# MarvinLvn/CPC2

Measured on AMD Instinct MI355X. Metric: audio-seconds/sec CPC training (1.28 s @16 kHz, 128 neg), higher is better.
Workload: dtype f32

## Files before the change

### cpc2_amd/_lib.py

```python
import ctypes
import os
import time

import torch

_HERE = os.path.dirname(os.path.abspath(__file__))
LIB_PATH = os.environ.get("CPC2_HIP_LIB") or os.path.join(_HERE, "libcpc2_hip.so")

c_float_p = ctypes.c_void_p
c_ptr = ctypes.c_void_p
c_int = ctypes.c_int
c_long = ctypes.c_long
c_size_t = ctypes.c_size_t
c_float = ctypes.c_float

SIGNATURES = {
    "cpc_version": (c_int, []),
    "cpc_last_error": (ctypes.c_char_p, []),
    "cpc_async_error_check": (c_int, [c_ptr]),
    "cpc_prof_enable": (c_int, [c_int]),
    "cpc_gemm_set_mode": (c_int, [c_int]),
    "cpc_prof_read": (c_int, [ctypes.c_char_p, ctypes.POINTER(ctypes.c_double), ctypes.POINTER(c_long)]),
    "cpc_gemm_nt": (c_int, [c_ptr, c_long, c_ptr, c_long, c_ptr, c_long, c_ptr, c_int, c_int, c_int, c_ptr]),
    "cpc_gemm_tn_scratch_bytes": (c_size_t, [c_int, c_int, c_long]),
# ... 51 lines not shown
    "cpc_mt_draw_host": (c_int, [c_ptr, c_ptr, c_size_t]),
    "cpc_mt_draw_host_async": (c_int, [c_ptr, c_ptr, c_size_t]),
    "cpc_mt_draw_device_async": (c_int, [c_ptr, c_ptr, c_ptr, c_size_t, c_int, c_ptr]),
    "cpc_mt_draw_expand_device_async": (c_int, [c_ptr, c_ptr, c_ptr, c_ptr, c_int, c_int, c_int, c_int, c_int, c_ptr]),
    "cpc_mt_redraw_expand_device_async": (c_int, [c_ptr, c_ptr, c_int, c_int, c_size_t, c_ptr, c_ptr, c_ptr, c_int, c_int, c_int, c_int, c_int, c_ptr]),
    "cpc_negidx_wait_on": (c_int, [c_ptr, c_ptr]),
    "cpc_negidx_stream": (c_int, [c_ptr, c_ptr]),
    "cpc_stream_create_apart": (c_int, [c_ptr, c_int, c_ptr]),
    "cpc_streams_overlap": (c_int, [c_ptr, c_ptr]),
    "cpc_stream_apart_failures": (c_long, []),
    "cpc_stream_spin": (c_int, [c_ptr, c_long]),
    "cpc_side_stream": (c_int, [c_ptr, c_ptr]),
    "cpc_negidx_expand": (c_int, [c_ptr, c_ptr, c_int, c_int, c_int, c_int, c_ptr]),
    "cpc_infonce_saved_bytes": (c_size_t, [c_int] * 6),
    "cpc_infonce_scratch_bytes": (c_size_t, [c_int] * 6),
    "cpc_infonce_logits_offset": (c_size_t, [c_int] * 6),
    "cpc_infonce_perm_offset": (c_size_t, [c_int] * 6),
    "cpc_infonce_forward": (c_int, [c_ptr] * 9 + [c_int] * 6 + [c_ptr]),
    "cpc_infonce_backward": (c_int, [c_ptr] * 11 + [c_int] * 6 + [c_ptr]),
    "cpc_infonce_backward_deferred": (c_int, [c_ptr] * 11 + [c_int] * 6 + [c_ptr]),
    "cpc_infonce_join": (c_int, [c_ptr]),
    "cpc_infonce_forward_cw": (c_int, [c_ptr] * 9 + [c_int] * 6 + [c_ptr]),
    "cpc_infonce_backward_cw": (c_int, [c_ptr] * 11 + [c_int] * 7 + [c_ptr]),
    "cpc_infonce_forward_pred": (c_int, [c_ptr] * 8 + [c_int] * 5 + [c_ptr]),
    "cpc_infonce_backward_pred": (c_int, [c_ptr] * 9 + [c_int] * 5 + [c_ptr]),
    "cpc_flac_info": (c_int, [ctypes.c_char_p, ctypes.POINTER(c_int), ctypes.POINTER(c_int), ctypes.POINTER(c_int),
                              ctypes.POINTER(c_long)]),
    "cpc_flac_decode_f32": (c_int, [ctypes.c_char_p, c_ptr, c_long, ctypes.POINTER(c_int)]),
    "cpc_window_gather": (c_int, [c_ptr, c_long, c_ptr, c_ptr, c_int, c_int, c_ptr]),
    "cpc_adam_step": (c_int, [c_ptr, c_ptr, c_ptr, c_ptr, c_long, c_int, c_float, c_float, c_float, c_float, c_float, c_ptr]),
# ... 121 lines not shown
```

### cpc2_amd/criterion.py

```python
import ctypes
import os

import numpy as np
import torch
import torch.nn as nn

from . import _lib
from ._lib import check, f32c, grad_buffers, ptr, require_gpu, scratch, stream_ptr


def _sleep_until(event):
    import time
    while not event.query():
        time.sleep(0.0001)


class NegativeSampler:

    RING = int(os.environ.get("CPC_SAMPLER_RING", "4"))

    def __init__(self):
        self._lib = _lib.load()
        self._h = ctypes.c_void_p(self._lib.cpc_mt_create(5489))
        if not self._h:
# ... 443 lines not shown
    def forward(ctx, z, ext_idx, weights, n_neg, *preds):
        require_gpu(z, ext_idx, weights, *preds)
        lib = _lib.load()
        z = f32c(z)
        preds = tuple(f32c(p) for p in preds)
        b, t, dim_enc = z.shape
        k = len(preds)
        if any(p.shape != (b, t - k, dim_enc) for p in preds):
            raise ValueError(f"predictions must be [b, W, dim_enc] = {(b, t - k, dim_enc)}")
        if ext_idx.dtype != torch.int32 or ext_idx.numel() != b * n_neg * (t - k):
            raise ValueError("ext_idx must be int32 [b, W, n_neg]")
        if weights is not None and weights.numel() != b * (t - k):
            raise ValueError(f"weights must hold one value per (window, frame): {b * (t - k)}, got {weights.numel()}")
        w = f32c(weights) if weights is not None else None
        nsaved = lib.cpc_infonce_saved_bytes(b, t, k, dim_enc, dim_enc, n_neg)
        nscratch = lib.cpc_infonce_scratch_bytes(b, t, k, dim_enc, dim_enc, n_neg)
        if nsaved == 0:
            check(-1, "infonce shape query")
        losses = torch.empty(k, dtype=torch.float32, device=z.device)
        acc = torch.empty(k, dtype=torch.float32, device=z.device)
        saved = torch.empty(nsaved, dtype=torch.uint8, device=z.device)
        sc = scratch(nscratch, z.device)
        check(lib.cpc_infonce_forward_pred(_lib.ptr_array(preds), ptr(z), ptr(ext_idx), ptr(w), ptr(losses), ptr(acc),
                                           ptr(saved), ptr(sc), b, t, k, dim_enc, n_neg, stream_ptr(z.device)),
              "infonce_forward_pred")
        ctx.save_for_backward(z, ext_idx, w, saved, *preds)
        ctx.dims = (b, t, k, dim_enc, n_neg)
        ctx.mark_non_differentiable(acc)
        ctx.set_materialize_grads(False)
        return losses, acc

    @staticmethod
    def backward(ctx, dlosses, _dacc):
        lib = _lib.load()
        z, ext_idx, w, saved, *preds = ctx.saved_tensors
        b, t, k, dim_enc, n_neg = ctx.dims
        if dlosses is None:
            dlosses = torch.zeros(k, dtype=torch.float32, device=z.device)
        dlosses = f32c(dlosses)
        dz = torch.empty_like(z)
        dpreds = [torch.empty_like(p) for p in preds]
        sc = scratch(lib.cpc_infonce_scratch_bytes(b, t, k, dim_enc, dim_enc, n_neg), z.device)
        check(lib.cpc_infonce_backward_pred(_lib.ptr_array(preds), ptr(z), ptr(ext_idx), ptr(w), ptr(dlosses), ptr(saved),
                                            ptr(sc), _lib.ptr_array(dpreds), ptr(dz), b, t, k, dim_enc, n_neg,
                                            stream_ptr(z.device)), "infonce_backward_pred")
        return (dz, None, None, None) + tuple(dpreds)


class _LinearFn(torch.autograd.Function):

    @staticmethod
    def forward(ctx, x, weight):
        require_gpu(x, weight)
        lib = _lib.load()
        x2 = f32c(x).reshape(-1, x.shape[-1])
        w = f32c(weight.detach())
        m, kdim = x2.shape
# ... 184 lines not shown
    def _logits(self, cFeature, encodedData, extIdx, n_neg):
        lib = _lib.load()
        with torch.no_grad():
            windowSize = cFeature.size(1) - self.nPredicts
            preds = self._predictions(cFeature[:, :windowSize].contiguous())
            z = f32c(encodedData)
            b, t, dim_enc = z.shape
            k = self.nPredicts
            losses = torch.empty(k, dtype=torch.float32, device=z.device)
            acc = torch.empty(k, dtype=torch.float32, device=z.device)
            dim_ar = dim_enc if preds is not None else cFeature.size(2)
            nsaved = lib.cpc_infonce_saved_bytes(b, t, k, dim_ar, dim_enc, n_neg)
            if nsaved == 0:
                check(-1, "infonce shape query")
            saved = torch.empty(nsaved, dtype=torch.uint8, device=z.device)
            sc = scratch(lib.cpc_infonce_scratch_bytes(b, t, k, dim_ar, dim_enc, n_neg), z.device)
            if preds is None:
                c = f32c(cFeature)
                wpred = torch.stack([f32c(p.weight.detach()) for p in self.wPrediction.predictors], dim=0)
                check(lib.cpc_infonce_forward(ptr(c), ptr(z), ptr(wpred), ptr(extIdx), None, ptr(losses), ptr(acc), ptr(saved),
                                              ptr(sc), b, t, k, dim_ar, dim_enc, n_neg, stream_ptr(z.device)), "infonce_forward")
            else:
                preds = [f32c(p) for p in preds]
                check(lib.cpc_infonce_forward_pred(_lib.ptr_array(preds), ptr(z), ptr(extIdx), None, ptr(losses), ptr(acc),
                                                   ptr(saved), ptr(sc), b, t, k, dim_enc, n_neg, stream_ptr(z.device)),
                      "infonce_forward_pred")
            off = lib.cpc_infonce_logits_offset(b, t, k, dim_ar, dim_enc, n_neg)
            n = b * windowSize * k * (n_neg + 1)
            slot_order = saved[off:off + 4 * n].view(torch.float32).view(b, windowSize, k, n_neg + 1)
            poff = lib.cpc_infonce_perm_offset(b, t, k, dim_ar, dim_enc, n_neg)
            perm = saved[poff:poff + 2 * b * windowSize * n_neg].view(torch.int16).view(b, windowSize, 1, n_neg).long() & 0xFFFF
# ... 246 lines not shown
```

### cpc2_amd/csrc/infonce.hip

```cpp
#include "common.h"
#include <hip/hip_ext.h>
#include "coop.h"
#include "ldsdma.h"
#include "rowcfg.h"

#include <algorithm>
#include <atomic>
#include <cstdlib>
#include <map>
#include <mutex>

namespace cpc {

typedef float f32x4 __attribute__((ext_vector_type(4)));
typedef float f32x16 __attribute__((ext_vector_type(16)));

constexpr int NCE_ROWS = 16;
constexpr int NCE_POS = 16;

struct NceArgs {
    const float *Pk[16];
    float *dPk[16];
    long p_stride;
    int p_rows;
    int p_packed;
    const float *z;
    const int32_t *ext;
    const unsigned short *perm;
    const float *weights;
    float *logits;
    float *lse;
    float *lossp;
    float *hit;
    int b, T, W, K, Nneg;
    int lw;
    const float *dloss;
    float *vbuf;
    float *ds_buf;
    float inv_count;
};

__global__ __launch_bounds__(64) void nce_block_sort_kernel(const int32_t *ext, int32_t *sorted, unsigned short *perm, int Nneg,
                                                            int rows_per_block, int nblk, int nrows, int *err)
{
    const long base = (long)blockIdx.x * Nneg;
    const int lane = threadIdx.x;
    int pos = 0;
    bool bad = false;
    for (int blk = 0; blk < nblk; ++blk)
        for (int c = 0; c < Nneg; c += 64) {
            const int j = c + lane;
            int row = j < Nneg ? ext[base + j] : -1;
            if (j < Nneg && (unsigned)row >= (unsigned)nrows) { bad = true; row = 0; }
// ... 483 lines not shown
#pragma unroll
        for (int dt = 0; dt < DT32; ++dt) {
            f32x16 acc;
#pragma unroll
            for (int e = 0; e < 16; ++e) acc[e] = 0.f;
#pragma unroll
            for (int kp = 0; kp < NCE_ROWS / 2; ++kp) acc = __builtin_amdgcn_mfma_f32_32x32x2f32(av[kp], bvals[dt][kp], acc, 0, 0, 0);
#pragma unroll
            for (int e = 0; e < 16; ++e)
                if (voff[e] >= 0) vb[voff[e] + dt * 32] = acc[e];
        }
    }
}

constexpr int NCE_SROW = 68;
template <int H, int NKK> __global__ __launch_bounds__(H / 2) void infonce_bwd_fused_kernel(NceArgs a)
{
    constexpr int NW = H / 128;
    extern __shared__ __attribute__((aligned(16))) float smem[];
    float *dS = smem;
    int *rowidx = reinterpret_cast<int *>(dS + NCE_ROWS * a.lw);
    float *stage0 = reinterpret_cast<float *>(rowidx + a.lw);
    const int wave = threadIdx.x >> 6, lane = threadIdx.x & 63, r = lane & 15, q = lane >> 4;
    float *stage = stage0 + wave * 16 * NCE_SROW;

    const int bb = blockIdx.x / a.p_rows, t = blockIdx.x - bb * a.p_rows;
    if (t >= a.W) {
        for (int k = 0; k < a.K; ++k) {
            float *row = a.dPk[k] + ((long)bb * a.p_rows + t) * a.p_stride;
            for (int i = threadIdx.x; i < H / 4; i += 64 * NW) reinterpret_cast<float4 *>(row)[i] = make_float4(0.f, 0.f, 0.f, 0.f);
        }
// ... 40 lines not shown
    }
    __syncthreads();
#pragma unroll
    for (int kk = 0; kk < KW; ++kk) {
        const int k = wave + NW * kk, kc = min(k, a.K - 1);
#pragma unroll
        for (int i = 0; i < GI; ++i) {
            const int g = lane + 64 * i;
            const float e = expf(stage0[kc * lrow + gi[i]] - lsek[kk]);
            float v = g >= NCE_POS ? (g < ncand ? coef[kk] * e : 0.f) : (g == k ? coef[kk] * (e - 1.f) : 0.f);
            if (k >= a.K) v = 0.f;
            if (g < a.lw) dS[k * a.lw + g] = v;
        }
    }
    __syncthreads();

    const int d0 = 128 * wave;
    const long prow_off = ((long)bb * a.p_rows + t) * a.p_stride + d0;
    float pa[8][NKK];
#pragma unroll
    for (int kk = 0; kk < NKK; ++kk) {
        const int k = 4 * kk + q;
        const float *pk = a.Pk[min(k, a.K - 1)] + prow_off + r;
#pragma unroll
        for (int tile = 0; tile < 8; ++tile) {
            const float v = pk[16 * tile];
            pa[tile][kk] = k < a.K ? v : 0.f;
        }
    }
    float *vb = a.vbuf + (bt * (long)ncand + q) * H + d0 + 4 * r;
#define NCE_ROWS_GROUP(C0)                                                                                                     \
    {                                                                                                                          \
        const int c0_ = (C0);                                                                                                  \
        float bv[NKK];                                                                                                         \
        _Pragma("unroll") for (int kk = 0; kk < NKK; ++kk) bv[kk] = dS[(4 * kk + q) * a.lw + c0_ + r];                        \
        _Pragma("unroll") for (int half = 0; half < 2; ++half) {                                                               \
            f32x4 acc[4];                                                                                                      \
            _Pragma("unroll") for (int tl = 0; tl < 4; ++tl) acc[tl] = (f32x4){0.f, 0.f, 0.f, 0.f};                            \
            _Pragma("unroll") for (int kk = 0; kk < NKK; ++kk)                                                                 \
                _Pragma("unroll") for (int tl = 0; tl < 4; ++tl)                                                               \
                    acc[tl] = __builtin_amdgcn_mfma_f32_16x16x4f32(pa[4 * half + tl][kk], bv[kk], acc[tl], 0, 0, 0);           \
            _Pragma("unroll") for (int tl = 0; tl < 4; ++tl)                                                                   \
                *reinterpret_cast<f32x4 *>(stage + r * NCE_SROW + 16 * tl + 4 * q) = acc[tl];                                  \
            __builtin_amdgcn_fence(__ATOMIC_RELEASE, "wavefront");                                                             \
            __builtin_amdgcn_wave_barrier();                                                                                   \
// ... 29 lines not shown
        auto multiply = [&](int buf) {
#pragma unroll
            for (int u = 0; u < 4; ++u)
#pragma unroll
                for (int T4 = 0; T4 < 2; ++T4) {
                    dp[T4][0] = __builtin_amdgcn_mfma_f32_16x16x4f32(av[buf][u][T4].x, bv4[buf][u], dp[T4][0], 0, 0, 0);
                    dp[T4][1] = __builtin_amdgcn_mfma_f32_16x16x4f32(av[buf][u][T4].y, bv4[buf][u], dp[T4][1], 0, 0, 0);
                    dp[T4][2] = __builtin_amdgcn_mfma_f32_16x16x4f32(av[buf][u][T4].z, bv4[buf][u], dp[T4][2], 0, 0, 0);
                    dp[T4][3] = __builtin_amdgcn_mfma_f32_16x16x4f32(av[buf][u][T4].w, bv4[buf][u], dp[T4][3], 0, 0, 0);
                }
        };
        const int nb = npad / 16;
        request(0, 0);
        for (int ib = 0; ib < nb; ib += 2) {
            request(1, 4 * (ib + 1));
            NCE_ROWS_GROUP(16 * ib)
            multiply(0);
            if (ib + 2 < nb) request(0, 4 * (ib + 2));
            if (16 * (ib + 1) < ncand) NCE_ROWS_GROUP(16 * (ib + 1))
            multiply(1);
        }
        if (r < a.K) {
            float *dprow = a.dPk[r] + ((long)bb * a.p_rows + t) * a.p_stride + d0;
#pragma unroll
            for (int T4 = 0; T4 < 2; ++T4)
#pragma unroll
                for (int reg = 0; reg < 4; ++reg)
                    *reinterpret_cast<float4 *>(dprow + 64 * T4 + 16 * q + 4 * reg) =
                        make_float4(dp[T4][0][reg], dp[T4][1][reg], dp[T4][2][reg], dp[T4][3][reg]);
        }
    }
#undef NCE_ROWS_GROUP
}

// ... 101 lines not shown
    }
    for (; e > beg; --e) {
        const int o = entries[e - 1];
        add_row((long)(o / Nneg) * vrows + pos_rows + o % Nneg);
    }
    for (int k = 0; k < K; ++k) {
        const int t = tp - 1 - k;
        if (t >= 0 && t < W) add_row(((long)bb * W + t) * vrows + k);
    }
#pragma unroll
    for (int c = 0; c < PER; ++c)
        if (lane + 64 * c < C4) reinterpret_cast<float4 *>(dz)[(long)r * C4 + lane + 64 * c] = acc[c];
    }
}

__global__ void negidx_expand_kernel(const uint32_t *raw, int32_t *ext, int b, int T, int W, int Nneg)
{
    const long n = (long)b * Nneg * W;
    for (long o = (long)blockIdx.x * blockDim.x + threadIdx.x; o < n; o += (long)gridDim.x * blockDim.x) {
        const int nn = (int)(o % Nneg);
        const long bt = o / Nneg;
        const int t = (int)(bt % W), bb = (int)(bt / W);
        const long i = ((long)bb * Nneg + nn) * W + t;
        const uint32_t bi = raw[i] % (uint32_t)b;
        uint32_t seq = raw[n + i] % (uint32_t)(T - 1) + 1u + (uint32_t)t;
        if (seq >= (uint32_t)T) seq -= (uint32_t)T;
        ext[o] = (int32_t)(seq + bi * (uint32_t)T);
    }
}

struct NceLayout {
    int b, T, K, W, Har, Henc, Nneg, lw;
    int Pr;
    float *P, *logits, *lse;
    int32_t *ext_sorted;
    unsigned short *perm;
    int nblk, rows_per_block;
    size_t saved_bytes;
    float *lossp, *hit, *dP, *wt, *tn, *tn_late;
    float *vbuf;
    float *ds_buf;
    int *counts, *offsets, *entries;
    size_t tn_bytes, scratch_bytes;
    size_t lds_fwd, lds_bwd, lds_bwd_fused;
};

static bool nce_supported(int H) { return H == 32 || H == 64 || H == 128 || H == 256 || H == 512; }

static int nce_layout(NceLayout &l, int b, int T, int K, int Har, int Henc, int Nneg, void *saved, void *scratch)
{
    CPC_REQUIRE(nce_supported(Henc), "infonce: encoder dim %d not supported (32, 64, 128, 256, 512)", Henc);
    CPC_REQUIRE(b > 0 && K >= 1 && K <= 16 && T > K && Nneg >= 1 && Har >= 1,
                "infonce: bad shape b=%d T=%d K=%d (1..16) dim_ar=%d n_neg=%d", b, T, K, Har, Nneg);
    l.b = b; l.T = T; l.K = K; l.W = T - K; l.Har = Har; l.Henc = Henc; l.Nneg = Nneg; l.Pr = T;
    l.lw = (int)cdiv(NCE_POS + Nneg, 32) * 32 + 4;
    Carver sv(saved);
    l.P = sv.take<float>((size_t)b * T * K * Henc);
    l.logits = sv.take<float>((size_t)b * l.W * K * (Nneg + 1));
    l.lse = sv.take<float>((size_t)b * l.W * K);
    l.ext_sorted = sv.take<int32_t>((size_t)b * l.W * Nneg);
    l.perm = sv.take<unsigned short>((size_t)b * l.W * Nneg + 1024);
    const size_t zbytes = sizeof(float) * (size_t)b * T * Henc;
    l.nblk = (int)std::min<size_t>(16, std::max<size_t>(1, (zbytes + (1u << 21) - 1) >> 21));
    l.rows_per_block = (int)cdiv((long)b * T, l.nblk);
    l.saved_bytes = sv.used();
    Carver sc(scratch);
    l.lossp = sc.take<float>((size_t)b * l.W * K);
    l.hit = sc.take<float>((size_t)b * l.W * K);
    l.dP = sc.take<float>((size_t)b * T * K * Henc);
    l.wt = sc.take<float>((size_t)K * Henc * Har);
    l.tn_bytes = std::max(gemm_tn_scratch_bytes(K * Henc, Har, (long)b * T), gemm_nt_scratch_bytes((long)b * T, Har, K * Henc));
    l.tn = sc.take<float>(l.tn_bytes / sizeof(float));
    l.tn_late = sc.take<float>(l.tn_bytes / sizeof(float));
    l.counts = sc.take<int>((size_t)b * T);
    l.offsets = sc.take<int>((size_t)b * T + 1);
    l.entries = sc.take<int>((size_t)b * l.W * Nneg);
    l.vbuf = sc.take<float>((size_t)b * l.W * (NCE_POS + Nneg) * Henc);
    l.ds_buf = sc.take<float>((size_t)b * l.W * (NCE_ROWS + 1) * l.lw);
    l.scratch_bytes = sc.used();
    l.lds_fwd = align_up(sizeof(int) * (size_t)Nneg + sizeof(unsigned short) * (size_t)Nneg, 16);
    l.lds_bwd = sizeof(float) * (size_t)NCE_ROWS * l.lw + sizeof(int) * (size_t)l.lw;
    CPC_REQUIRE(l.lds_bwd <= 64 * 1024, "infonce: n_neg=%d needs %zu B of LDS (> 64 KiB)", Nneg, l.lds_bwd);
    l.lds_bwd_fused = l.lds_bwd + sizeof(float) * (size_t)(Henc / 128) * 16 * NCE_SROW;
    return CPC_OK;
}

template <typename Kern> static int allow_lds(Kern kern, size_t bytes)
{
    if (bytes > 64 * 1024)
        CPC_CHECK_HIP(hipFuncSetAttribute(reinterpret_cast<const void *>(kern), hipFuncAttributeMaxDynamicSharedMemorySize, (int)bytes));
    return CPC_OK;
}
// ... 87 lines not shown
    std::lock_guard<std::mutex> lk(mu);
    NceSide &sd = sides[dev];
    if (sd.stream == nullptr) {
        CPC_TRY(stream_create_apart(&caller, 1, &sd.stream));
        CPC_CHECK_HIP(hipEventCreateWithFlags(&sd.fork, hipEventDisableTiming));
        CPC_CHECK_HIP(hipEventCreateWithFlags(&sd.join, hipEventDisableTiming));
        CPC_CHECK_HIP(hipEventCreateWithFlags(&sd.mid, hipEventDisableTiming));
        CPC_CHECK_HIP(hipEventCreateWithFlags(&sd.late, hipEventDisableTiming));
        CPC_CHECK_HIP(hipEventCreateWithFlags(&sd.tail_fork, hipEventDisableTiming));
        CPC_CHECK_HIP(hipEventCreateWithFlags(&sd.tail, hipEventDisableTiming));
    }
    *out = &sd;
    return CPC_OK;
}

static int nce_launch_gather(const NceLayout &l, float *dz, bool fused, hipStream_t st)
{
    const int rows = l.b * l.T;
    const unsigned wgs = (unsigned)cdiv(rows, 4);
    NCE_DISPATCH(l.Henc, hipLaunchKernelGGL(infonce_dz_gather_kernel<HH>, dim3(wgs), dim3(256), 0, st, l.vbuf,
                                             l.offsets, l.entries, dz, l.b, l.T, l.W, l.K, l.Nneg, fused ? NCE_POS : l.K));
    CPC_CHECK_LAUNCH("infonce_dz_gather_kernel");
    return CPC_OK;
}

static int nce_launch_bwd(NceArgs &a, const NceLayout &l, float *dz, hipStream_t st, NceSide **late = nullptr)
{
    const long n = (long)l.b * l.W * l.Nneg;
    const int rows = l.b * l.T;
    a.vbuf = l.vbuf;
    a.ds_buf = l.ds_buf;
    ProfScope prof(PROF_NCE_BWD, st);
    NceSide *side = nullptr;
    CPC_TRY(nce_side(&side, st));
    CPC_CHECK_HIP(hipEventRecord(side->fork, st));
    CPC_CHECK_HIP(hipStreamWaitEvent(side->stream, side->fork, 0));
    const unsigned blocks = (unsigned)std::min<long>(cdiv(n, 256), 4096);
    CPC_CHECK_HIP(hipMemsetAsync(l.counts, 0, sizeof(int) * (size_t)rows, side->stream));
    hipLaunchKernelGGL(nce_hist_kernel, dim3(blocks), dim3(256), 0, side->stream, a.ext, n, l.counts);
    hipLaunchKernelGGL(nce_scan_kernel, dim3(1), dim3(1024), 0, side->stream, l.counts, rows, l.offsets);
    CPC_CHECK_HIP(hipMemsetAsync(l.counts, 0, sizeof(int) * (size_t)rows, side->stream));
    hipLaunchKernelGGL(nce_fill_kernel, dim3(blocks), dim3(256), 0, side->stream, a.ext, n, l.offsets, l.counts, l.entries);
    hipLaunchKernelGGL(nce_sort_kernel, dim3((unsigned)cdiv(rows, 4)), dim3(256), 0, side->stream, l.offsets, l.entries, rows);
    CPC_CHECK_LAUNCH("infonce reference lists");
    CPC_CHECK_HIP(hipEventRecord(side->join, side->stream));
    int status = CPC_OK;
    const bool fused = (l.Henc == 256 || l.Henc == 512) && a.perm != nullptr && l.lw <= 320 &&
                       l.Nneg % 16 == 0 && (size_t)l.K * (l.Nneg + 1) <= (size_t)(l.Henc / 128) * 16 * NCE_SROW;
    if (fused) {
        const unsigned grid = (unsigned)(l.b * a.p_rows);
#define NCE_FUSED(HH, NKK)                                                                                                  \
    {                                                                                                                       \
        status = allow_lds(infonce_bwd_fused_kernel<HH, NKK>, l.lds_bwd_fused);                                             \
        if (status == CPC_OK) hipLaunchKernelGGL((infonce_bwd_fused_kernel<HH, NKK>), dim3(grid), dim3(HH / 2), l.lds_bwd_fused, st, a); \
    }
        const int nkk = (l.K + 3) / 4;
        if (l.Henc == 256) {
            if (nkk == 1) NCE_FUSED(256, 1) else if (nkk == 2) NCE_FUSED(256, 2) else if (nkk == 3) NCE_FUSED(256, 3) else NCE_FUSED(256, 4)
        } else {
            if (nkk == 1) NCE_FUSED(512, 1) else if (nkk == 2) NCE_FUSED(512, 2) else if (nkk == 3) NCE_FUSED(512, 3) else NCE_FUSED(512, 4)
        }
#undef NCE_FUSED
    } else {
        NCE_DISPATCH(l.Henc, {
// ... 1 lines not shown
            if (status == CPC_OK) hipLaunchKernelGGL(infonce_bwd_kernel<HH>, dim3((unsigned)(l.b * a.p_rows)), dim3(64), l.lds_bwd, st, a);
        });
    }
    CPC_TRY(status);
    CPC_CHECK_LAUNCH("infonce_bwd_kernel");
    if (!fused) {
        NCE_DISPATCH(l.Henc, hipLaunchKernelGGL(infonce_dz_store_kernel<HH>, dim3((unsigned)(l.b * l.W)), dim3(64), l.lds_bwd, st, a));
        CPC_CHECK_LAUNCH("infonce_dz_store_kernel");
    }
    if (late != nullptr) {
        *late = side;
        side->late_fused = fused;
        return CPC_OK;
    }
    CPC_CHECK_HIP(hipStreamWaitEvent(st, side->join, 0));
    CPC_TRY(nce_launch_gather(l, dz, fused, st));
    return CPC_OK;
}

static int infonce_forward(const float *c, const float *z, const float *wpred, const int32_t *ext, const float *weights,
                           float *losses, float *acc, void *saved, void *scratch, int b, int T, int K, int Har, int Henc,
                           int Nneg, hipStream_t st, int c_frames = 0)
{
    NceLayout l;
    CPC_TRY(nce_layout(l, b, T, K, Har, Henc, Nneg, saved, scratch));
    if (c_frames != 0) {
        CPC_REQUIRE(c_frames == T || c_frames == l.W, "infonce: the context holds %d frames per window (expected %d or %d)", c_frames, T, l.W);
        l.Pr = c_frames;
    }
    RowMap none{};
    CPC_TRY(gemm_nt(c, Har, wpred, Har, l.P, (long)K * Henc, nullptr, (long)b * l.Pr, K * Henc, Har, none, st));
    CPC_TRY(nce_sort_negatives(l, ext, st));
    NceArgs a{};
    nce_common(a, l, z, ext, weights);
    for (int k = 0; k < K; ++k) a.Pk[k] = l.P + (size_t)k * Henc;
    a.p_stride = (long)K * Henc; a.p_rows = l.Pr;
    a.p_packed = (size_t)b * T * K * Henc * sizeof(float) < (1ull << 32) ? 1 : 0;
    return nce_launch_fwd(a, l, losses, acc, st);
}

static int infonce_backward(const float *c, const float *z, const float *wpred, const int32_t *ext, const float *weights,
                            const float *dlosses, void *saved, void *scratch, float *dc, float *dz, float *dwpred, int b, int T,
                            int K, int Har, int Henc, int Nneg, hipStream_t st, bool defer, int c_frames = 0)
{
    NceLayout l;
    CPC_TRY(nce_layout(l, b, T, K, Har, Henc, Nneg, saved, scratch));
    if (c_frames != 0) {
        CPC_REQUIRE(c_frames == T || c_frames == l.W, "infonce: the context holds %d frames per window (expected %d or %d)", c_frames, T, l.W);
        l.Pr = c_frames;
    }
    NceArgs a{};
    nce_common(a, l, z, ext, weights);
    for (int k = 0; k < K; ++k) { a.Pk[k] = l.P + (size_t)k * Henc; a.dPk[k] = l.dP + (size_t)k * Henc; }
    a.p_stride = (long)K * Henc; a.p_rows = l.Pr;
    a.dloss = dlosses;
    NceSide *late = nullptr;
    CPC_TRY(nce_launch_bwd(a, l, dz, st, defer ? &late : nullptr));
    CPC_TRY(transpose2d(wpred, l.wt, K * Henc, Har, st));
    RowMap none{};
    none.splitk_scratch = l.tn; none.splitk_bytes = l.tn_bytes;
    CPC_TRY(gemm_nt(l.dP, (long)K * Henc, l.wt, (long)K * Henc, dc, Har, nullptr, (long)b * l.Pr, Har, K * Henc, none, st));
    if (late != nullptr) {
        late->l = l; late->dz = dz; late->dwpred = dwpred; late->c = c;
        late->started = false; late->marked = false;
        late->pending.store(true);
    } else {
        CPC_TRY(gemm_tn(l.dP, (long)K * Henc, c, Har, dwpred, Har, K * Henc, Har, (long)b * l.Pr, l.tn, l.tn_bytes, 0, 0, st));
    }
    return CPC_OK;
}
// ... 4 lines not shown
    CPC_TRY(nce_side(&side, st));
    if (!side->pending.load() || side->started || side->marked) return CPC_OK;
    CPC_CHECK_HIP(hipEventRecord(side->mid, st));
    side->marked = true;
    return CPC_OK;
}

int infonce_deferred_start(hipStream_t st)
{
    NceSide *side = nullptr;
    CPC_TRY(nce_side(&side, st));
    if (!side->pending.load() || side->started) return CPC_OK;
    const NceLayout &l = side->l;
    CPC_TRY(infonce_deferred_mark(st));
    CPC_CHECK_HIP(hipStreamWaitEvent(side->stream, side->mid, 0));
    CPC_TRY(nce_launch_gather(l, side->dz, side->late_fused, side->stream));
    CPC_TRY(gemm_tn(l.dP, (long)l.K * l.Henc, side->c, l.Har, side->dwpred, l.Har, l.K * l.Henc, l.Har, (long)l.b * l.Pr, l.tn_late, l.tn_bytes, 0,
                    0, side->stream));
    CPC_CHECK_HIP(hipEventRecord(side->late, side->stream));
    side->started = true;
    return CPC_OK;
}

int side_tail_begin(hipStream_t st, hipStream_t *side_stream)
{
    NceSide *side = nullptr;
    CPC_TRY(nce_side(&side, st));
    CPC_CHECK_HIP(hipEventRecord(side->tail_fork, st));
    CPC_CHECK_HIP(hipStreamWaitEvent(side->stream, side->tail_fork, 0));
    *side_stream = side->stream;
    return CPC_OK;
// ... 41 lines not shown
    if (side->pending.load()) {
        CPC_TRY(infonce_deferred_start(st));
        {
            ProfScope held(PROF_SIDE_WAIT, st);
            CPC_CHECK_HIP(hipStreamWaitEvent(st, side->late, 0));
        }
        side->pending.store(false);
    }
    return CPC_OK;
}

static int infonce_forward_pred(const float *const *pred, const float *z, const int32_t *ext, const float *weights, float *losses,
                                float *acc, void *saved, void *scratch, int b, int T, int K, int Henc, int Nneg, hipStream_t st)
{
    NceLayout l;
    CPC_TRY(nce_layout(l, b, T, K, Henc, Henc, Nneg, saved, scratch));
    CPC_TRY(nce_sort_negatives(l, ext, st));
    NceArgs a{};
    nce_common(a, l, z, ext, weights);
    for (int k = 0; k < K; ++k) a.Pk[k] = pred[k];
    a.p_stride = Henc; a.p_rows = l.W;
    return nce_launch_fwd(a, l, losses, acc, st);
}

static int infonce_backward_pred(const float *const *pred, const float *z, const int32_t *ext, const float *weights,
                                 const float *dlosses, void *saved, void *scratch, float *const *dpred, float *dz, int b, int T, int K,
                                 int Henc, int Nneg, hipStream_t st)
{
    NceLayout l;
    CPC_TRY(nce_layout(l, b, T, K, Henc, Henc, Nneg, saved, scratch));
    NceArgs a{};
    nce_common(a, l, z, ext, weights);
    for (int k = 0; k < K; ++k) { a.Pk[k] = pred[k]; a.dPk[k] = dpred[k]; }
    a.p_stride = Henc; a.p_rows = l.W;
    a.dloss = dlosses;
    return nce_launch_bwd(a, l, dz, st);
}

}

extern "C" int cpc_negidx_expand(const uint32_t *raw, int32_t *ext_idx, int batch, int seq_len, int window, int n_neg,
                                 cpc_stream_t stream)
{
    CPC_REQUIRE(raw != nullptr && ext_idx != nullptr && batch >= 1 && seq_len >= 2 && window >= 1 && window <= seq_len && n_neg >= 1 &&
                    (long long)batch * seq_len <= 2147483647LL,
                "cpc_negidx_expand: bad arguments (batch=%d seq_len=%d window=%d n_neg=%d)", batch, seq_len, window, n_neg);
    const long n = (long)batch * n_neg * window;
    hipLaunchKernelGGL(cpc::negidx_expand_kernel, dim3((unsigned)std::min<long>(cpc::cdiv(n, 256), 2048)), dim3(256), 0,
                       static_cast<hipStream_t>(stream), raw, ext_idx, batch, seq_len, window, n_neg);
    CPC_CHECK_LAUNCH("negidx_expand_kernel");
    return CPC_OK;
}

extern "C" size_t cpc_infonce_saved_bytes(int b, int t, int k, int dim_ar, int dim_enc, int n_neg)
{
    cpc::NceLayout l;
    if (cpc::nce_layout(l, b, t, k, dim_ar, dim_enc, n_neg, nullptr, nullptr) != CPC_OK) return 0;
    return l.saved_bytes;
}

extern "C" size_t cpc_infonce_logits_offset(int b, int t, int k, int dim_ar, int dim_enc, int n_neg)
{
    cpc::NceLayout l;
    char *const base = reinterpret_cast<char *>(4096);
    if (cpc::nce_layout(l, b, t, k, dim_ar, dim_enc, n_neg, base, nullptr) != CPC_OK) return (size_t)-1;
    return (size_t)(reinterpret_cast<char *>(l.logits) - base);
}

extern "C" size_t cpc_infonce_perm_offset(int b, int t, int k, int dim_ar, int dim_enc, int n_neg)
{
    cpc::NceLayout l;
    char *const base = reinterpret_cast<char *>(4096);
    if (cpc::nce_layout(l, b, t, k, dim_ar, dim_enc, n_neg, base, nullptr) != CPC_OK) return (size_t)-1;
    return (size_t)(reinterpret_cast<char *>(l.perm) - base);
}

extern "C" size_t cpc_infonce_scratch_bytes(int b, int t, int k, int dim_ar, int dim_enc, int n_neg)
{
    cpc::NceLayout l;
    if (cpc::nce_layout(l, b, t, k, dim_ar, dim_enc, n_neg, nullptr, nullptr) != CPC_OK) return 0;
    return l.scratch_bytes;
}

extern "C" int cpc_infonce_forward(const float *c, const float *z, const float *wpred, const int32_t *ext_idx, const float *weights,
                                   float *losses, float *acc, void *saved, void *scratch, int b, int t, int k, int dim_ar,
                                   int dim_enc, int n_neg, cpc_stream_t stream)
{
    return cpc::infonce_forward(c, z, wpred, ext_idx, weights, losses, acc, saved, scratch, b, t, k, dim_ar, dim_enc, n_neg,
                                static_cast<hipStream_t>(stream));
}

extern "C" int cpc_infonce_backward(const float *c, const float *z, const float *wpred, const int32_t *ext_idx, const float *weights,
                                    const float *dlosses, void *saved, void *scratch, float *dc, float *dz, float *dwpred, int b,
                                    int t, int k, int dim_ar, int dim_enc, int n_neg, cpc_stream_t stream)
{
// ... 55 lines not shown
```

### include/cpc2_hip.h

```cpp
#ifndef CPC2_HIP_H
#define CPC2_HIP_H

#include <stddef.h>
#include <stdint.h>

#ifdef __cplusplus
extern "C" {
#endif

typedef void *cpc_stream_t;

enum cpc_status {
    CPC_OK = 0,
    CPC_ERR_INVALID = -1,
    CPC_ERR_HIP = -2,
    CPC_ERR_WORKSPACE = -3
};

int cpc_version(void);
const char *cpc_last_error(void);

int cpc_async_error_check(cpc_stream_t stream);

int cpc_stream_create_apart(const cpc_stream_t *avoid, int n_avoid, cpc_stream_t *out);
// ... 139 lines not shown
                         float *dc, float *dz, float *dwpred, int b, int t, int k, int dim_ar,
                         int dim_enc, int n_neg, cpc_stream_t stream);
int cpc_infonce_backward_deferred(const float *c, const float *z, const float *wpred, const int32_t *ext_idx,
                                  const float *weights, const float *dlosses, void *saved, void *scratch,
                                  float *dc, float *dz, float *dwpred, int b, int t, int k, int dim_ar,
                                  int dim_enc, int n_neg, cpc_stream_t stream);
int cpc_infonce_join(cpc_stream_t stream);
int cpc_infonce_forward_cw(const float *c, const float *z, const float *wpred, const int32_t *ext_idx,
                           const float *weights, float *losses, float *acc, void *saved, void *scratch,
                           int b, int t, int k, int dim_ar, int dim_enc, int n_neg, cpc_stream_t stream);
int cpc_infonce_backward_cw(const float *c, const float *z, const float *wpred, const int32_t *ext_idx,
                            const float *weights, const float *dlosses, void *saved, void *scratch,
                            float *dc, float *dz, float *dwpred, int b, int t, int k, int dim_ar,
                            int dim_enc, int n_neg, int deferred, cpc_stream_t stream);

int cpc_infonce_forward_pred(const float *const *pred, const float *z, const int32_t *ext_idx, const float *weights,
                             float *losses, float *acc, void *saved, void *scratch, int b, int t, int k,
                             int dim_enc, int n_neg, cpc_stream_t stream);
int cpc_infonce_backward_pred(const float *const *pred, const float *z, const int32_t *ext_idx,
                              const float *weights, const float *dlosses, void *saved, void *scratch,
                              float *const *dpred, float *dz, int b, int t, int k, int dim_enc, int n_neg,
                              cpc_stream_t stream);

int cpc_flac_info(const char *path, int *sample_rate, int *channels, int *bits_per_sample,
                  long *total_samples);
int cpc_flac_decode_f32(const char *path, float *out_host, long capacity_floats, int *md5_ok);

int cpc_window_gather(const float *audio, long total_samples, const long *offsets, float *out, int batch,
                      int window, cpc_stream_t stream);

// ... 51 lines not shown
```

Measured before the change: 17700.

## Compute InfoNCE dz via context-space accumulation and a GEMM instead of materialized vbuf

```diff
diff --git a/cpc2_amd/_lib.py b/cpc2_amd/_lib.py
--- a/cpc2_amd/_lib.py
+++ b/cpc2_amd/_lib.py
@@ -89,6 +89,7 @@
     "cpc_negidx_expand": (c_int, [c_ptr, c_ptr, c_int, c_int, c_int, c_int, c_ptr]),
     "cpc_infonce_saved_bytes": (c_size_t, [c_int] * 6),
     "cpc_infonce_scratch_bytes": (c_size_t, [c_int] * 6),
+    "cpc_infonce_pred_scratch_bytes": (c_size_t, [c_int] * 5),
     "cpc_infonce_logits_offset": (c_size_t, [c_int] * 6),
     "cpc_infonce_perm_offset": (c_size_t, [c_int] * 6),
     "cpc_infonce_forward": (c_int, [c_ptr] * 9 + [c_int] * 6 + [c_ptr]),
diff --git a/cpc2_amd/criterion.py b/cpc2_amd/criterion.py
--- a/cpc2_amd/criterion.py
+++ b/cpc2_amd/criterion.py
@@ -481,7 +481,7 @@
             raise ValueError(f"weights must hold one value per (window, frame): {b * (t - k)}, got {weights.numel()}")
         w = f32c(weights) if weights is not None else None
         nsaved = lib.cpc_infonce_saved_bytes(b, t, k, dim_enc, dim_enc, n_neg)
-        nscratch = lib.cpc_infonce_scratch_bytes(b, t, k, dim_enc, dim_enc, n_neg)
+        nscratch = lib.cpc_infonce_pred_scratch_bytes(b, t, k, dim_enc, n_neg)
         if nsaved == 0:
             check(-1, "infonce shape query")
         losses = torch.empty(k, dtype=torch.float32, device=z.device)
@@ -507,7 +507,7 @@
         dlosses = f32c(dlosses)
         dz = torch.empty_like(z)
         dpreds = [torch.empty_like(p) for p in preds]
-        sc = scratch(lib.cpc_infonce_scratch_bytes(b, t, k, dim_enc, dim_enc, n_neg), z.device)
+        sc = scratch(lib.cpc_infonce_pred_scratch_bytes(b, t, k, dim_enc, n_neg), z.device)
         check(lib.cpc_infonce_backward_pred(_lib.ptr_array(preds), ptr(z), ptr(ext_idx), ptr(w), ptr(dlosses), ptr(saved),
                                             ptr(sc), _lib.ptr_array(dpreds), ptr(dz), b, t, k, dim_enc, n_neg,
                                             stream_ptr(z.device)), "infonce_backward_pred")
@@ -722,7 +722,8 @@
             if nsaved == 0:
                 check(-1, "infonce shape query")
             saved = torch.empty(nsaved, dtype=torch.uint8, device=z.device)
-            sc = scratch(lib.cpc_infonce_scratch_bytes(b, t, k, dim_ar, dim_enc, n_neg), z.device)
+            sc = scratch(lib.cpc_infonce_scratch_bytes(b, t, k, dim_ar, dim_enc, n_neg) if preds is None
+                         else lib.cpc_infonce_pred_scratch_bytes(b, t, k, dim_enc, n_neg), z.device)
             if preds is None:
                 c = f32c(cFeature)
                 wpred = torch.stack([f32c(p.weight.detach()) for p in self.wPrediction.predictors], dim=0)
diff --git a/cpc2_amd/csrc/infonce.hip b/cpc2_amd/csrc/infonce.hip
--- a/cpc2_amd/csrc/infonce.hip
+++ b/cpc2_amd/csrc/infonce.hip
@@ -37,6 +37,7 @@
     const float *dloss;
     float *vbuf;
     float *ds_buf;
+    float *dst;
     float inv_count;
 };
 
@@ -550,7 +551,7 @@
 }
 
 constexpr int NCE_SROW = 68;
-template <int H, int NKK> __global__ __launch_bounds__(H / 2) void infonce_bwd_fused_kernel(NceArgs a)
+template <int H, int NKK, bool CTX = false> __global__ __launch_bounds__(H / 2) void infonce_bwd_fused_kernel(NceArgs a)
 {
     constexpr int NW = H / 128;
     extern __shared__ __attribute__((aligned(16))) float smem[];
@@ -621,12 +622,23 @@
         }
     }
     __syncthreads();
+    if constexpr (CTX) {
+        float *drow = a.dst + bt * (long)ncand * 16;
+        for (int i = threadIdx.x; i < 4 * ncand; i += 64 * NW) {
+            const int cand = i >> 2, k4 = 4 * (i & 3);
+            const int g = cand;
+            *reinterpret_cast<float4 *>(drow + 4 * i) = make_float4(dS[k4 * a.lw + g], dS[(k4 + 1) * a.lw + g], dS[(k4 + 2) * a.lw + g],
+                                                                    dS[(k4 + 3) * a.lw + g]);
+        }
+        if (blockIdx.x == 0 && threadIdx.x < 4)
+            reinterpret_cast<float4 *>(a.dst + (long)a.b * a.W * ncand * 16)[threadIdx.x] = make_float4(0.f, 0.f, 0.f, 0.f);
+    }
 
     const int d0 = 128 * wave;
     const long prow_off = ((long)bb * a.p_rows + t) * a.p_stride + d0;
     float pa[8][NKK];
 #pragma unroll
-    for (int kk = 0; kk < NKK; ++kk) {
+    for (int kk = 0; kk < (CTX ? 0 : NKK); ++kk) {
         const int k = 4 * kk + q;
         const float *pk = a.Pk[min(k, a.K - 1)] + prow_off + r;
 #pragma unroll
@@ -635,7 +647,7 @@
             pa[tile][kk] = k < a.K ? v : 0.f;
         }
     }
-    float *vb = a.vbuf + (bt * (long)ncand + q) * H + d0 + 4 * r;
+    float *vb = CTX ? nullptr : a.vbuf + (bt * (long)ncand + q) * H + d0 + 4 * r;
 #define NCE_ROWS_GROUP(C0)                                                                                                     \
     {                                                                                                                          \
         const int c0_ = (C0);                                                                                                  \
@@ -695,10 +707,12 @@
         request(0, 0);
         for (int ib = 0; ib < nb; ib += 2) {
             request(1, 4 * (ib + 1));
-            NCE_ROWS_GROUP(16 * ib)
+            if constexpr (!CTX) NCE_ROWS_GROUP(16 * ib)
             multiply(0);
             if (ib + 2 < nb) request(0, 4 * (ib + 2));
-            if (16 * (ib + 1) < ncand) NCE_ROWS_GROUP(16 * (ib + 1))
+            if constexpr (!CTX) {
+                if (16 * (ib + 1) < ncand) NCE_ROWS_GROUP(16 * (ib + 1))
+            }
             multiply(1);
         }
         if (r < a.K) {
@@ -830,6 +844,102 @@
     }
 }
 
+template <int H> __global__ __launch_bounds__(256, 8) void infonce_dz_ctx_kernel(const float *dst, const float *c, const int *offsets,
+                                                                                const int *entries, float *U, int rows, int T, int W,
+                                                                                int K, int Nneg, int Pr)
+{
+    constexpr int NWR = H / 128;
+    static_assert(NWR == 1 || NWR == 2 || NWR == 4, "a workgroup of four waves holds whole rows");
+    const int wave = __builtin_amdgcn_readfirstlane(threadIdx.x >> 6), lane = threadIdx.x & 63, r = lane & 15, q = lane >> 4;
+    const int row = blockIdx.x * (4 / NWR) + wave / NWR;
+    if (row >= rows) return;
+    const unsigned d0b = (unsigned)(128 * (wave % NWR) + 4 * r) * 4u;
+    const int bb = row / T, tp = row - bb * T;
+    const int beg = offsets[row], nlist = offsets[row + 1] - beg, ntot = nlist + K;
+    const unsigned ncand = (unsigned)(NCE_POS + Nneg);
+    const char *const cb = reinterpret_cast<const char *>(c), *const db = reinterpret_cast<const char *>(dst);
+
+    f32x4 acc[2][4];
+#pragma unroll
+    for (int T4 = 0; T4 < 2; ++T4)
+#pragma unroll
+        for (int e = 0; e < 4; ++e) acc[T4][e] = (f32x4){0.f, 0.f, 0.f, 0.f};
+
+    for (int base = 0; base < ntot; base += 64) {
+        const int j = base + lane;
+        unsigned coef = (unsigned)(rows / T * W) * ncand;
+        unsigned crow = 0;
+        if (j < nlist) {
+            const unsigned o = (unsigned)entries[beg + j];
+            const unsigned bt = o / (unsigned)Nneg, slot = o - bt * (unsigned)Nneg;
+            const unsigned wb = bt / (unsigned)W;
+            coef = bt * ncand + NCE_POS + slot;
+            crow = wb * (unsigned)Pr + (bt - wb * (unsigned)W);
+        } else if (j < ntot) {
+            const int k = j - nlist, t = tp - 1 - k;
+            if (t >= 0 && t < W) {
+                coef = (unsigned)(bb * W + t) * ncand + (unsigned)k;
+                crow = (unsigned)(bb * Pr + t);
+            }
+        }
+        crow *= (unsigned)(H * 4);
+        coef *= 64u;
+        const int ng = (min(64, ntot - base) + 3) >> 2;
+        float4 av[2][2];
+        float bv[2];
+        auto request = [&](int buf, int g) {
+            const int from = 4 * g + q;
+            const unsigned co = __shfl(crow, from, 64) + d0b;
+            bv[buf] = *reinterpret_cast<const float *>(db + (__shfl(coef, from, 64) + 4u * r));
+            av[buf][0] = *reinterpret_cast<const float4 *>(cb + co);
+            av[buf][1] = *reinterpret_cast<const float4 *>(cb + co + 256u);
+        };
+        auto multiply = [&](int buf) {
+            const float bvv = bv[buf];
+#pragma unroll
+            for (int T4 = 0; T4 < 2; ++T4) {
+                acc[T4][0] = __builtin_amdgcn_mfma_f32_16x16x4f32(av[buf][T4].x, bvv, acc[T4][0], 0, 0, 0);
+                acc[T4][1] = __builtin_amdgcn_mfma_f32_16x16x4f32(av[buf][T4].y, bvv, acc[T4][1], 0, 0, 0);
+                acc[T4][2] = __builtin_amdgcn_mfma_f32_16x16x4f32(av[buf][T4].z, bvv, acc[T4][2], 0, 0, 0);
+                acc[T4][3] = __builtin_amdgcn_mfma_f32_16x16x4f32(av[buf][T4].w, bvv, acc[T4][3], 0, 0, 0);
+            }
+        };
+        request(0, 0);
+        request(1, 1);
+        for (int g = 0; g < ng; g += 2) {
+            __builtin_amdgcn_sched_barrier(0);
+            multiply(0);
+            __builtin_amdgcn_sched_barrier(0);
+            request(0, (g + 2) & 15);
+            __builtin_amdgcn_sched_barrier(0);
+            multiply(1);
+            __builtin_amdgcn_sched_barrier(0);
+            request(1, (g + 3) & 15);
+        }
+    }
+    if (r < K) {
+        float *u = U + ((long)row * K + r) * H + 128 * (wave % NWR) + 16 * q;
+#pragma unroll
+        for (int T4 = 0; T4 < 2; ++T4)
+#pragma unroll
+            for (int reg = 0; reg < 4; ++reg)
+                *reinterpret_cast<float4 *>(u + 64 * T4 + 4 * reg) =
+                    make_float4(acc[T4][0][reg], acc[T4][1][reg], acc[T4][2][reg], acc[T4][3][reg]);
+    }
+}
+
+__global__ void nce_wperm_kernel(const float *wpred, float *wperm, int K, int Henc, int Har)
+{
+    const long n4 = (long)K * Henc * Har / 4;
+    const int h4 = Har / 4;
+    for (long i = (long)blockIdx.x * blockDim.x + threadIdx.x; i < n4; i += (long)gridDim.x * blockDim.x) {
+        const int a4 = (int)(i % h4);
+        const long ke = i / h4;
+        const int e = (int)(ke % Henc), k = (int)(ke / Henc);
+        reinterpret_cast<float4 *>(wperm)[((long)e * K + k) * h4 + a4] = reinterpret_cast<const float4 *>(wpred)[i];
+    }
+}
+
 __global__ void negidx_expand_kernel(const uint32_t *raw, int32_t *ext, int b, int T, int W, int Nneg)
 {
     const long n = (long)b * Nneg * W;
@@ -856,6 +966,11 @@
     float *lossp, *hit, *dP, *wt, *tn, *tn_late;
     float *vbuf;
     float *ds_buf;
+    bool ctx;
+    float *dst;
+    float *U;
+    float *wperm;
+    const float *c_in, *w_in;
     int *counts, *offsets, *entries;
     size_t tn_bytes, scratch_bytes;
     size_t lds_fwd, lds_bwd, lds_bwd_fused;
@@ -863,7 +978,12 @@
 
 static bool nce_supported(int H) { return H == 32 || H == 64 || H == 128 || H == 256 || H == 512; }
 
-static int nce_layout(NceLayout &l, int b, int T, int K, int Har, int Henc, int Nneg, void *saved, void *scratch)
+static bool nce_fused_shape(int K, int Henc, int Nneg, int lw)
+{
+    return (Henc == 256 || Henc == 512) && lw <= 320 && Nneg % 16 == 0 && (size_t)K * (Nneg + 1) <= (size_t)(Henc / 128) * 16 * NCE_SROW;
+}
+
+static int nce_layout(NceLayout &l, int b, int T, int K, int Har, int Henc, int Nneg, void *saved, void *scratch, bool linear)
 {
     CPC_REQUIRE(nce_supported(Henc), "infonce: encoder dim %d not supported (32, 64, 128, 256, 512)", Henc);
     CPC_REQUIRE(b > 0 && K >= 1 && K <= 16 && T > K && Nneg >= 1 && Har >= 1,
@@ -886,12 +1006,23 @@
     l.dP = sc.take<float>((size_t)b * T * K * Henc);
     l.wt = sc.take<float>((size_t)K * Henc * Har);
     l.tn_bytes = std::max(gemm_tn_scratch_bytes(K * Henc, Har, (long)b * T), gemm_nt_scratch_bytes((long)b * T, Har, K * Henc));
+    l.ctx = linear && nce_fused_shape(K, Henc, Nneg, l.lw) && (Har == 256 || Har == 512) &&
+            sizeof(float) * (size_t)b * T * Har < (1ull << 32) && 64 * ((size_t)b * l.W * (NCE_POS + Nneg) + 1) < (1ull << 32);
+    l.c_in = nullptr; l.w_in = nullptr;
+    if (l.ctx) l.tn_bytes = std::max(l.tn_bytes, gemm_nt_scratch_bytes((long)b * T, Henc, K * Har));
     l.tn = sc.take<float>(l.tn_bytes / sizeof(float));
     l.tn_late = sc.take<float>(l.tn_bytes / sizeof(float));
     l.counts = sc.take<int>((size_t)b * T);
     l.offsets = sc.take<int>((size_t)b * T + 1);
     l.entries = sc.take<int>((size_t)b * l.W * Nneg);
-    l.vbuf = sc.take<float>((size_t)b * l.W * (NCE_POS + Nneg) * Henc);
+    l.vbuf = nullptr; l.dst = nullptr; l.U = nullptr; l.wperm = nullptr;
+    if (l.ctx) {
+        l.dst = sc.take<float>(((size_t)b * l.W * (NCE_POS + Nneg) + 1) * 16);
+        l.U = sc.take<float>((size_t)b * T * K * Har);
+        l.wperm = sc.take<float>((size_t)K * Henc * Har);
+    } else {
+        l.vbuf = sc.take<float>((size_t)b * l.W * (NCE_POS + Nneg) * Henc);
+    }
     l.ds_buf = sc.take<float>((size_t)b * l.W * (NCE_ROWS + 1) * l.lw);
     l.scratch_bytes = sc.used();
     l.lds_fwd = align_up(sizeof(int) * (size_t)Nneg + sizeof(unsigned short) * (size_t)Nneg, 16);
@@ -1009,9 +1140,26 @@
     return CPC_OK;
 }
 
-static int nce_launch_gather(const NceLayout &l, float *dz, bool fused, hipStream_t st)
+static int nce_launch_gather(const NceLayout &l, float *dz, bool fused, hipStream_t st, float *tn)
 {
     const int rows = l.b * l.T;
+    if (l.ctx) {
+        CPC_REQUIRE(fused && l.c_in != nullptr && l.w_in != nullptr, "infonce: context form of dz without its inputs");
+        if (l.Har == 256)
+            hipLaunchKernelGGL(infonce_dz_ctx_kernel<256>, dim3((unsigned)cdiv(rows, 2)), dim3(256), 0, st, l.dst, l.c_in, l.offsets, l.entries,
+                               l.U, rows, l.T, l.W, l.K, l.Nneg, l.Pr);
+        else
+            hipLaunchKernelGGL(infonce_dz_ctx_kernel<512>, dim3((unsigned)rows), dim3(256), 0, st, l.dst, l.c_in, l.offsets, l.entries, l.U,
+                               rows, l.T, l.W, l.K, l.Nneg, l.Pr);
+        CPC_CHECK_LAUNCH("infonce_dz_ctx_kernel");
+        const long n4 = (long)l.K * l.Henc * l.Har / 4;
+        hipLaunchKernelGGL(nce_wperm_kernel, dim3((unsigned)std::min<long>(cdiv(n4, 256), 2048)), dim3(256), 0, st, l.w_in, l.wperm, l.K,
+                           l.Henc, l.Har);
+        CPC_CHECK_LAUNCH("nce_wperm_kernel");
+        RowMap none{};
+        none.splitk_scratch = tn; none.splitk_bytes = l.tn_bytes;
+        return gemm_nt(l.U, (long)l.K * l.Har, l.wperm, (long)l.K * l.Har, dz, l.Henc, nullptr, rows, l.Henc, l.K * l.Har, none, st);
+    }
     const unsigned wgs = (unsigned)cdiv(rows, 4);
     NCE_DISPATCH(l.Henc, hipLaunchKernelGGL(infonce_dz_gather_kernel<HH>, dim3(wgs), dim3(256), 0, st, l.vbuf,
                                              l.offsets, l.entries, dz, l.b, l.T, l.W, l.K, l.Nneg, fused ? NCE_POS : l.K));
@@ -1025,6 +1173,7 @@
     const int rows = l.b * l.T;
     a.vbuf = l.vbuf;
     a.ds_buf = l.ds_buf;
+    a.dst = l.dst;
     ProfScope prof(PROF_NCE_BWD, st);
     NceSide *side = nullptr;
     CPC_TRY(nce_side(&side, st));
@@ -1040,9 +1189,18 @@
     CPC_CHECK_LAUNCH("infonce reference lists");
     CPC_CHECK_HIP(hipEventRecord(side->join, side->stream));
     int status = CPC_OK;
-    const bool fused = (l.Henc == 256 || l.Henc == 512) && a.perm != nullptr && l.lw <= 320 &&
-                       l.Nneg % 16 == 0 && (size_t)l.K * (l.Nneg + 1) <= (size_t)(l.Henc / 128) * 16 * NCE_SROW;
-    if (fused) {
+    const bool fused = nce_fused_shape(l.K, l.Henc, l.Nneg, l.lw) && a.perm != nullptr;
+    CPC_REQUIRE(fused || !l.ctx, "infonce: context form of dz without the fused backward");
+    if (fused && l.ctx) {
+        const unsigned grid = (unsigned)(l.b * a.p_rows);
+        if (l.Henc == 256) {
+            status = allow_lds(infonce_bwd_fused_kernel<256, 1, true>, l.lds_bwd_fused);
+            if (status == CPC_OK) hipLaunchKernelGGL((infonce_bwd_fused_kernel<256, 1, true>), dim3(grid), dim3(128), l.lds_bwd_fused, st, a);
+        } else {
+            status = allow_lds(infonce_bwd_fused_kernel<512, 1, true>, l.lds_bwd_fused);
+            if (status == CPC_OK) hipLaunchKernelGGL((infonce_bwd_fused_kernel<512, 1, true>), dim3(grid), dim3(256), l.lds_bwd_fused, st, a);
+        }
+    } else if (fused) {
         const unsigned grid = (unsigned)(l.b * a.p_rows);
 #define NCE_FUSED(HH, NKK)                                                                                                  \
     {                                                                                                                       \
@@ -1074,7 +1232,7 @@
         return CPC_OK;
     }
     CPC_CHECK_HIP(hipStreamWaitEvent(st, side->join, 0));
-    CPC_TRY(nce_launch_gather(l, dz, fused, st));
+    CPC_TRY(nce_launch_gather(l, dz, fused, st, l.tn));
     return CPC_OK;
 }
 
@@ -1083,7 +1241,7 @@
                            int Nneg, hipStream_t st, int c_frames = 0)
 {
     NceLayout l;
-    CPC_TRY(nce_layout(l, b, T, K, Har, Henc, Nneg, saved, scratch));
+    CPC_TRY(nce_layout(l, b, T, K, Har, Henc, Nneg, saved, scratch, true));
     if (c_frames != 0) {
         CPC_REQUIRE(c_frames == T || c_frames == l.W, "infonce: the context holds %d frames per window (expected %d or %d)", c_frames, T, l.W);
         l.Pr = c_frames;
@@ -1104,7 +1262,7 @@
                             int K, int Har, int Henc, int Nneg, hipStream_t st, bool defer, int c_frames = 0)
 {
     NceLayout l;
-    CPC_TRY(nce_layout(l, b, T, K, Har, Henc, Nneg, saved, scratch));
+    CPC_TRY(nce_layout(l, b, T, K, Har, Henc, Nneg, saved, scratch, true));
     if (c_frames != 0) {
         CPC_REQUIRE(c_frames == T || c_frames == l.W, "infonce: the context holds %d frames per window (expected %d or %d)", c_frames, T, l.W);
         l.Pr = c_frames;
@@ -1114,6 +1272,7 @@
     for (int k = 0; k < K; ++k) { a.Pk[k] = l.P + (size_t)k * Henc; a.dPk[k] = l.dP + (size_t)k * Henc; }
     a.p_stride = (long)K * Henc; a.p_rows = l.Pr;
     a.dloss = dlosses;
+    l.c_in = c; l.w_in = wpred;
     NceSide *late = nullptr;
     CPC_TRY(nce_launch_bwd(a, l, dz, st, defer ? &late : nullptr));
     CPC_TRY(transpose2d(wpred, l.wt, K * Henc, Har, st));
@@ -1148,7 +1307,7 @@
     const NceLayout &l = side->l;
     CPC_TRY(infonce_deferred_mark(st));
     CPC_CHECK_HIP(hipStreamWaitEvent(side->stream, side->mid, 0));
-    CPC_TRY(nce_launch_gather(l, side->dz, side->late_fused, side->stream));
+    CPC_TRY(nce_launch_gather(l, side->dz, side->late_fused, side->stream, l.tn_late));
     CPC_TRY(gemm_tn(l.dP, (long)l.K * l.Henc, side->c, l.Har, side->dwpred, l.Har, l.K * l.Henc, l.Har, (long)l.b * l.Pr, l.tn_late, l.tn_bytes, 0,
                     0, side->stream));
     CPC_CHECK_HIP(hipEventRecord(side->late, side->stream));
@@ -1220,7 +1379,7 @@
                                 float *acc, void *saved, void *scratch, int b, int T, int K, int Henc, int Nneg, hipStream_t st)
 {
     NceLayout l;
-    CPC_TRY(nce_layout(l, b, T, K, Henc, Henc, Nneg, saved, scratch));
+    CPC_TRY(nce_layout(l, b, T, K, Henc, Henc, Nneg, saved, scratch, false));
     CPC_TRY(nce_sort_negatives(l, ext, st));
     NceArgs a{};
     nce_common(a, l, z, ext, weights);
@@ -1234,7 +1393,7 @@
                                  int Henc, int Nneg, hipStream_t st)
 {
     NceLayout l;
-    CPC_TRY(nce_layout(l, b, T, K, Henc, Henc, Nneg, saved, scratch));
+    CPC_TRY(nce_layout(l, b, T, K, Henc, Henc, Nneg, saved, scratch, false));
     NceArgs a{};
     nce_common(a, l, z, ext, weights);
     for (int k = 0; k < K; ++k) { a.Pk[k] = pred[k]; a.dPk[k] = dpred[k]; }
@@ -1261,7 +1420,7 @@
 extern "C" size_t cpc_infonce_saved_bytes(int b, int t, int k, int dim_ar, int dim_enc, int n_neg)
 {
     cpc::NceLayout l;
-    if (cpc::nce_layout(l, b, t, k, dim_ar, dim_enc, n_neg, nullptr, nullptr) != CPC_OK) return 0;
+    if (cpc::nce_layout(l, b, t, k, dim_ar, dim_enc, n_neg, nullptr, nullptr, true) != CPC_OK) return 0;
     return l.saved_bytes;
 }
 
@@ -1269,7 +1428,7 @@
 {
     cpc::NceLayout l;
     char *const base = reinterpret_cast<char *>(4096);
-    if (cpc::nce_layout(l, b, t, k, dim_ar, dim_enc, n_neg, base, nullptr) != CPC_OK) return (size_t)-1;
+    if (cpc::nce_layout(l, b, t, k, dim_ar, dim_enc, n_neg, base, nullptr, true) != CPC_OK) return (size_t)-1;
     return (size_t)(reinterpret_cast<char *>(l.logits) - base);
 }
 
@@ -1277,14 +1436,21 @@
 {
     cpc::NceLayout l;
     char *const base = reinterpret_cast<char *>(4096);
-    if (cpc::nce_layout(l, b, t, k, dim_ar, dim_enc, n_neg, base, nullptr) != CPC_OK) return (size_t)-1;
+    if (cpc::nce_layout(l, b, t, k, dim_ar, dim_enc, n_neg, base, nullptr, true) != CPC_OK) return (size_t)-1;
     return (size_t)(reinterpret_cast<char *>(l.perm) - base);
 }
 
 extern "C" size_t cpc_infonce_scratch_bytes(int b, int t, int k, int dim_ar, int dim_enc, int n_neg)
 {
     cpc::NceLayout l;
-    if (cpc::nce_layout(l, b, t, k, dim_ar, dim_enc, n_neg, nullptr, nullptr) != CPC_OK) return 0;
+    if (cpc::nce_layout(l, b, t, k, dim_ar, dim_enc, n_neg, nullptr, nullptr, true) != CPC_OK) return 0;
+    return l.scratch_bytes;
+}
+
+extern "C" size_t cpc_infonce_pred_scratch_bytes(int b, int t, int k, int dim_enc, int n_neg)
+{
+    cpc::NceLayout l;
+    if (cpc::nce_layout(l, b, t, k, dim_enc, dim_enc, n_neg, nullptr, nullptr, false) != CPC_OK) return 0;
     return l.scratch_bytes;
 }
 
diff --git a/include/cpc2_hip.h b/include/cpc2_hip.h
--- a/include/cpc2_hip.h
+++ b/include/cpc2_hip.h
@@ -177,6 +177,7 @@
                             float *dc, float *dz, float *dwpred, int b, int t, int k, int dim_ar,
                             int dim_enc, int n_neg, int deferred, cpc_stream_t stream);
 
+size_t cpc_infonce_pred_scratch_bytes(int b, int t, int k, int dim_enc, int n_neg);
 int cpc_infonce_forward_pred(const float *const *pred, const float *z, const int32_t *ext_idx, const float *weights,
                              float *losses, float *acc, void *saved, void *scratch, int b, int t, int k,
                              int dim_enc, int n_neg, cpc_stream_t stream);
```

Result: no change. 18010, median of 6 (+1.8%).
